# hassony2/homan

Measured on AMD Instinct MI355X. Metric: optimisation iters/sec (30-frame 256^2 clip), higher is better.
Workload: dtype f32

## Files before the change

homan_amd/csrc/raster_fwd.hip:

```cpp
#include "raster_ws.h"

#ifdef RASTER_TRACE
#define RASTER_TRACE_WGS 65536
__device__ unsigned g_raster_trace[RASTER_TRACE_WGS][9];
__device__ int g_raster_trace_F = 0, g_raster_trace_depth = -1;
#define RPH_MARK(k) do { if (tid == 0) { const unsigned long long t_ = wall_clock64(); rtr[k] += (unsigned)(t_ - rtr_t); rtr_t = t_; } } while (0)
#elif defined(RASTER_PHASES)
__device__ unsigned long long g_raster_ph[24];
#define RPH_MARK(k) do { if (tid == 0) { const unsigned long long t_ = clock64(); rph[k] += t_ - rph_t; rph_t = t_; } } while (0)
#else
#define RPH_MARK(k)
#endif
#ifndef CAND_CAP
#define CAND_CAP 512
#endif
#ifndef RB_PASS
#define RB_PASS 128
#endif
#ifndef HM_PRUNE
#define HM_PRUNE 1
#endif
#ifndef RASTER_WPE
#define RASTER_WPE 6
#endif
__device__ __forceinline__ void raster_fwd_body(
    const int blk, const float* __restrict__ faces9, const FaceBox* __restrict__ boxes, int B, int F, int S, float znear,
    float zfar, int* __restrict__ idx_map, unsigned short* __restrict__ alpha16, float* __restrict__ pooled,
    const float* __restrict__ keep, const float* __restrict__ ref, float* __restrict__ dimg,
    float* __restrict__ partials, const int* __restrict__ work_order, unsigned char* __restrict__ owned,
    float* __restrict__ pooled_depth, unsigned short* __restrict__ planes,
    int* __restrict__ bin_cnt, const int* __restrict__ bin_list, unsigned int* __restrict__ done, int reset_bins,
    unsigned char* __restrict__ region_state, int persistent, float* __restrict__ alpha_full, int mask_shared,
    float* __restrict__ dimg_full, const unsigned int* __restrict__ hint, unsigned long long* __restrict__ ts_slots,
    int* __restrict__ wo_dyn, unsigned int* __restrict__ wg_cost)
{
    const unsigned long long ts_t0 = (unsigned long long)wall_clock64();
    __shared__ unsigned long long zb[32 * 32];
    __shared__ int cand[2 * CAND_CAP];
    __shared__ float4 recs[RB_PASS][5];
    __shared__ int ustart[RB_PASS];
    __shared__ unsigned czn[RB_PASS];
    __shared__ unsigned hz[64];
    __shared__ unsigned short uq[RASTER_WAVES][128];
    __shared__ int wsum[RASTER_WAVES];
    __shared__ int cand_n[2];
    const int w = __builtin_amdgcn_readfirstlane((int)(threadIdx.x >> 6)), lane = threadIdx.x & 63, tid = threadIdx.x;
    const int is = 2 * S, tiles_x = S / HM_TILE, ntiles = tiles_x * tiles_x, regions_x = tiles_x / 2;
    const bool dyn = wo_dyn && hint[2] != 0u;
    const int wo = __builtin_amdgcn_readfirstlane(dyn ? wo_dyn[blk]
                                                     : work_order ? work_order[blk] : (int)(((blk % B) << 16) | (blk / B)));
    if (wo_dyn && !dyn && threadIdx.x == 0) wo_dyn[blk] = wo;
    const int region = wo & 0xffff, b = wo >> 16;
    const int rx = region % regions_x, ry = region / regions_x;
    const int tx = 2 * rx + (w & 1), ty = 2 * ry + (w >> 1);
    const int tile = ty * tiles_x + tx;

    const int gx0 = rx * 2 * HM_STILE, gx1 = gx0 + 2 * HM_STILE - 1;
    const int gy1 = is - 1 - ry * 2 * HM_STILE, gy0 = gy1 - (2 * HM_STILE - 1);
    const float gcx0 = (float)(2 * gx0 + 1 - is) / (float)is, gcx1 = (float)(2 * gx1 + 1 - is) / (float)is;
    const float gcy0 = (float)(2 * gy0 + 1 - is) / (float)is, gcy1 = (float)(2 * gy1 + 1 - is) / (float)is;
    const bool pow2 = (is & (is - 1)) == 0;
    const float inv_is = 1.0f / (float)is;
    const unsigned long long zb_empty = ((unsigned long long)__float_as_uint(zfar) << 32) | 0xffffffffull;

    int had_any = 0;
    const uint2* bx = reinterpret_cast<const uint2*>(boxes) + (long)b * F;
    const int nsx = (is + (1 << hm_sr_shift(is)) - 1) >> hm_sr_shift(is);
    const int sr = (gy0 >> hm_sr_shift(is)) * nsx + (gx0 >> hm_sr_shift(is));
    unsigned char* rstate = region_state + (long)b * regions_x * regions_x + region;
    const int nscan = bin_cnt ? bin_cnt[b * nsx * nsx + sr] : F;
    const int rstate0 = persistent ? (int)*rstate : 0;
    const int* scan = bin_cnt ? bin_list + ((long)b * nsx * nsx + sr) * F : nullptr;
    const bool idle = nscan == 0 && rstate0 == 1;
    const bool ts_on = hm_ts_enabled(hint) && tid == 0;
    if (ts_on) hm_ts_store(ts_slots, blk, 0, ts_t0);
#ifdef RASTER_TRACE
    unsigned rtr[6] = {0, 0, 0, 0, 0, 0}, rtr_cand = 0, rtr_units = 0;
    unsigned long long rtr_t = ts_t0;
#endif
#ifdef RASTER_PHASES
    unsigned long long rph[6] = {0, 0, 0, 0, 0, 0}, rph_t = clock64();
    unsigned long long rph_units[3] = {0, 0, 0};
    unsigned rph_pairs = 0;
    __shared__ unsigned s_rph_iters;
    if (tid == 0) s_rph_iters = 0u;
    __syncthreads();
#endif
    if (!idle) {
#pragma unroll
        for (int k = 0; k < 4; ++k) zb[tid + 256 * k] = zb_empty;
    }
    const int near_w = hint ? (int)(hint[0] & 1u) : 0;
    auto unit_body = [&](const int i, const int k) {
        const float4 r0 = recs[i][0], r1 = recs[i][1], r4 = recs[i][4];
        const int fn = __float_as_int(r4.z), pk = __float_as_int(r4.w);
        const int nbx = (pk >> 6) & 15;
        const int kby = (k * (pk >> 10)) >> 16;
        const int sx0 = 4 * ((pk & 7) + (k - kby * nbx)), sy0 = 4 * (((pk >> 3) & 7) + kby);
        float Xs[4], Ys[4];
#pragma unroll
        for (int j = 0; j < 4; ++j) {
            const int xi = gx0 + sx0 + j, yi = gy0 + sy0 + j;
            const float xn = (float)(2 * xi + 1 - is), yn = (float)(2 * yi + 1 - is);
            Xs[j] = pow2 ? xn * inv_is : xn / (float)is;
            Ys[j] = pow2 ? yn * inv_is : yn / (float)is;
        }
        unsigned acc[16];
        {
            const float vx[3] = {r0.x, r0.z, r1.x}, vy[3] = {r0.y, r0.w, r1.y};
#pragma unroll
            for (int e = 0; e < 3; ++e) {
                const int e1 = e == 2 ? 0 : e + 1;
                const float ex = vx[e1] - vx[e], ey = vy[e1] - vy[e];
                float rv[4], cv[4];
#pragma unroll
                for (int j = 0; j < 4; ++j) { rv[j] = (Ys[j] - vy[e]) * ex + 0.0f; cv[j] = (Xs[j] - vx[e]) * ey; }
#pragma unroll
                for (int idx = 0; idx < 16; ++idx) {
                    const unsigned d = __float_as_uint(rv[idx >> 2] - cv[idx & 3]);
                    acc[idx] = e ? (acc[idx] | d) : d;
                }
#pragma unroll
                for (int idx = 0; idx < 16; ++idx) asm volatile("" : "+v"(acc[idx]));
            }
        }
        unsigned outside = 0u;
#pragma unroll
        for (int idx = 15; idx >= 0; --idx) outside = __builtin_amdgcn_alignbit(outside, acc[idx], 31);
        unsigned inside = ~outside & 0xffffu;
        if (inside == 0u) return;
#if HM_PRUNE
        {
            const unsigned zn = czn[i];
#pragma unroll
            for (int j = 0; j < 4; ++j) {
                if (((inside >> (4 * j)) & 0xfu) == 0u) continue;
                const uint4 ka = *reinterpret_cast<const uint4*>(&zb[(sy0 + j) * 32 + sx0]);
                const uint4 kb = *reinterpret_cast<const uint4*>(&zb[(sy0 + j) * 32 + sx0 + 2]);
                unsigned keepm = (zn > ka.y ? 0u : 1u) | (zn > ka.w ? 0u : 2u) | (zn > kb.y ? 0u : 4u) | (zn > kb.w ? 0u : 8u);
                inside &= ~(0xfu << (4 * j)) | (keepm << (4 * j));
            }
            if (inside == 0u) return;
        }
#endif
#ifdef RASTER_PHASES
        rph_pairs += __popc(inside);
        {
            const unsigned mx = (unsigned)hm_wave_max((float)__popc(inside));
            if (lane == __ffsll((long long)__ballot(1)) - 1) atomicAdd(&s_rph_iters, mx);
        }
#endif
        const float4 r2 = recs[i][2], r3 = recs[i][3];
        const float rz0 = r1.z, rz1 = r1.w, rz2 = r2.x;
        const float iv[9] = {r2.y, r2.z, r2.w, r3.x, r3.y, r3.z, r3.w, r4.x, r4.y};
        const int xb = gx0 + sx0, yb = gy0 + sy0;
        while (inside) {
            const int sidx = __ffs((int)inside) - 1;
            inside &= inside - 1;
            const int j = sidx >> 2, c4 = sidx & 3;
            const float xf = (float)(xb + c4), yf = (float)(yb + j);
            float wgt[3], ws = 0.0f;
#pragma unroll
            for (int q = 0; q < 3; ++q) {
                float t = iv[3 * q] * xf;
                t = t + iv[3 * q + 1] * yf;
                t = t + iv[3 * q + 2];
                t = fminf(fmaxf(t, 0.0f), 1.0f);
                wgt[q] = t;
                ws += t;
            }
            float sum = wgt[0] * rz0;
            sum = sum + wgt[1] * rz1;
            sum = sum + wgt[2] * rz2;
            const float zp = ws / sum;
            if (zp > znear && zp < zfar)
                atomicMin(&zb[(sy0 + j) * 32 + sx0 + c4],
                          ((unsigned long long)__float_as_uint(zp) << 32) | (unsigned)fn);
        }
    };
    for (int cbase = 0; cbase < nscan; cbase += CAND_CAP) {
        if (tid == 0) { cand_n[0] = 0; cand_n[1] = 0; }
        __syncthreads();
        uint2 v[CAND_CAP / 256];
        int vf[CAND_CAP / 256];
#pragma unroll
        for (int k = 0; k < CAND_CAP / 256; ++k) {
            const int e = cbase + k * 256 + tid;
            vf[k] = e < nscan ? (scan ? scan[e] : e) : -1;
        }
#pragma unroll
        for (int k = 0; k < CAND_CAP / 256; ++k) v[k] = vf[k] >= 0 ? bx[vf[k]] : make_uint2(0u, 0u);
#pragma unroll
        for (int k = 0; k < CAND_CAP / 256; ++k) {
            const int fi = vf[k];
            const int x0 = v[k].x & 0x3fff, y0 = (int)(v[k].x >> 16), x1 = (int)(v[k].y & 0xffff), y1 = (int)(v[k].y >> 16);
            const unsigned m = (x1 < gx0 || x0 > gx1 || y1 < gy0 || y0 > gy1) ? 0u : ((v[k].x >> 14) & 3u);
#pragma unroll
            for (int var = 0; var < 2; ++var) {
                const bool hit = (m >> var) & 1u;
                const unsigned long long bal = __ballot(hit);
                if (bal == 0ull) continue;
                const int cls = var == near_w ? 0 : 1;
                int basep = 0;
                if (lane == 0) basep = atomicAdd(&cand_n[cls], __popcll(bal));
                basep = __builtin_amdgcn_readfirstlane(basep);
                const int at = basep + __popcll(bal & ((1ull << lane) - 1ull));
                if (hit) cand[cls ? 2 * CAND_CAP - 1 - at : at] = fi | (var << 30);
            }
        }
        __syncthreads();
        RPH_MARK(0);
        had_any |= cand_n[0] | cand_n[1];
        const int n_near = cand_n[0], n_far = cand_n[1];
        for (int e0 = 0; e0 < n_near || e0 < n_far; e0 += RB_PASS / 2) {
            int units = 0;
            const int cls = tid >> 6, ci = e0 + (tid & 63);
            if (tid < RB_PASS && ci < (cls ? n_far : n_near)) {
                const int e = cand[cls ? 2 * CAND_CAP - 1 - ci : ci];
                const int fi = e & 0x3fffffff, var = e >> 30;
                const float* src = faces9 + ((long)b * F + fi) * 9;
                const uint2 u = bx[fi];
                float f[9];
                if (var == 0) {
#pragma unroll
                    for (int k = 0; k < 9; ++k) f[k] = src[k];
                } else {
#pragma unroll
                    for (int k = 0; k < 3; ++k) { f[3 * k] = src[3 * (2 - k)]; f[3 * k + 1] = src[3 * (2 - k) + 1]; f[3 * k + 2] = src[3 * (2 - k) + 2]; }
                }
                float p[3][2];
#pragma unroll
                for (int k = 0; k < 3; ++k) { p[k][0] = topix(f[3 * k], is); p[k][1] = topix(f[3 * k + 1], is); }
                const float inv[9] = {
                    p[1][1] - p[2][1], p[2][0] - p[1][0], p[1][0] * p[2][1] - p[2][0] * p[1][1],
                    p[2][1] - p[0][1], p[0][0] - p[2][0], p[2][0] * p[0][1] - p[0][0] * p[2][1],
                    p[0][1] - p[1][1], p[1][0] - p[0][0], p[0][0] * p[1][1] - p[1][0] * p[0][1]};
                const float den = p[2][0] * (p[0][1] - p[1][1]) + p[0][0] * (p[1][1] - p[2][1]) +
                                  p[1][0] * (p[2][1] - p[0][1]);
                bool miss = (den == 0.0f);
#pragma unroll
                for (int k = 0; k < 3; ++k) {
                    const int k1 = (k + 1) % 3;
                    const float ax = f[3 * k], ay = f[3 * k + 1], ex = f[3 * k1] - ax, ey = f[3 * k1 + 1] - ay;
                    bool all_out = true;
                    float mag = 0.f;
                    float lhs[4], rhs[4];
#pragma unroll
                    for (int cnr = 0; cnr < 4; ++cnr) {
                        const float X = (cnr & 1) ? gcx1 : gcx0, Y = (cnr & 2) ? gcy1 : gcy0;
                        lhs[cnr] = (Y - ay) * ex;
                        rhs[cnr] = (X - ax) * ey;
                        mag = fmaxf(mag, fabsf(lhs[cnr]) + fabsf(rhs[cnr]));
                    }
#pragma unroll
                    for (int cnr = 0; cnr < 4; ++cnr) all_out = all_out && (lhs[cnr] < rhs[cnr] - 1e-5f * mag);
                    miss = miss || all_out;
                }
                if (!miss) {
                    const int x0 = u.x & 0x3fff, y0 = (int)(u.x >> 16), x1 = (int)(u.y & 0xffff), y1 = (int)(u.y >> 16);
                    const int bx0 = (max(x0, gx0) - gx0) >> 2, bx1 = (min(x1, gx1) - gx0) >> 2;
                    const int by0 = (max(y0, gy0) - gy0) >> 2, by1 = (min(y1, gy1) - gy0) >> 2;
                    const int nbx = bx1 - bx0 + 1;
                    units = nbx * (by1 - by0 + 1);
                    const float rz0 = 1.0f / f[2], rz1 = 1.0f / f[5], rz2 = 1.0f / f[8];
                    recs[tid][0] = make_float4(f[0], f[1], f[3], f[4]);
                    recs[tid][1] = make_float4(f[6], f[7], rz0, rz1);
                    recs[tid][2] = make_float4(rz2, inv[0] / den, inv[1] / den, inv[2] / den);
                    recs[tid][3] = make_float4(inv[3] / den, inv[4] / den, inv[5] / den, inv[6] / den);
                    recs[tid][4] = make_float4(inv[7] / den, inv[8] / den, __int_as_float(fi + var * F),
                                               __int_as_float(bx0 | (by0 << 3) | (nbx << 6) | (((0x10000 + nbx - 1) / nbx) << 10)));
                    czn[tid] = __float_as_uint((1.0f / fmaxf(rz0, fmaxf(rz1, rz2))) * (1.0f - 1e-5f));
                }
            }
            const int incl = hm_wave_scan_incl(units);
            if (lane == 63 && w < 2) wsum[w] = incl;
            if (tid < RB_PASS) ustart[tid] = incl - units;
            __syncthreads();
            const int total_near = wsum[0], total_far = wsum[1];
#ifdef RASTER_TRACE
            rtr_cand += (unsigned)min(n_near - e0, RB_PASS / 2) * (e0 < n_near) + ((unsigned)min(n_far - e0, RB_PASS / 2) * (e0 < n_far) << 16);
            rtr_units += (unsigned)total_near + ((unsigned)total_far << 16);
#endif
#ifdef RASTER_PHASES
            if (tid < RB_PASS && ci < (cls ? n_far : n_near)) atomicAdd(&g_raster_ph[12 + cls], 1ull);
            rph_units[0] += total_near;
            rph_units[1] += total_far;
#endif
            RPH_MARK(1);
            for (int u = tid; u < total_near; u += 256) {
                int i = 0;
#pragma unroll
                for (int stp = RB_PASS / 4; stp > 0; stp >>= 1)
                    if (ustart[i + stp] <= u) i += stp;
                unit_body(i, u - ustart[i]);
            }
            RPH_MARK(2);
            if (total_far > 0) {
                if (tid < 64) hz[tid] = 0u;
                __syncthreads();
                {
                    const int blk = tid >> 2, row = (blk >> 3) * 4 + (tid & 3), col0 = (blk & 7) * 4;
                    const uint4 ka = *reinterpret_cast<const uint4*>(&zb[row * 32 + col0]);
                    const uint4 kb = *reinterpret_cast<const uint4*>(&zb[row * 32 + col0 + 2]);
                    atomicMax(&hz[blk], max(max(ka.y, ka.w), max(kb.y, kb.w)));
                }
                __syncthreads();
                RPH_MARK(3);
                int qn = 0;
                for (int u0 = 64 * w; u0 < total_far; u0 += 256) {
                    const int u = u0 + lane;
                    bool pass = false;
                    int ent = 0;
                    if (u < total_far) {
                        int i = 0;
#pragma unroll
                        for (int stp = RB_PASS / 4; stp > 0; stp >>= 1)
                            if (ustart[RB_PASS / 2 + i + stp] <= u) i += stp;
                        i += RB_PASS / 2;
                        const int k = u - ustart[i];
                        const int pk = __float_as_int(recs[i][4].w);
                        const int nbx = (pk >> 6) & 15, kby = (k * (pk >> 10)) >> 16;
                        const int blk = (((pk >> 3) & 7) + kby) * 8 + (pk & 7) + (k - kby * nbx);
                        pass = !(czn[i] > hz[blk]);
                        ent = i | (k << 8);
                    }
                    const unsigned long long bal = __ballot(pass);
#ifdef RASTER_PHASES
                    if (lane == 0) atomicAdd(&g_raster_ph[21], (unsigned long long)__popcll(bal));
#endif
                    if (pass) uq[w][qn + __popcll(bal & ((1ull << lane) - 1ull))] = (unsigned short)ent;
                    qn += __popcll(bal);
                    wave_sync();
                    if (qn >= 64) {
                        qn -= 64;
                        const int e = uq[w][qn + lane];
                        wave_sync();
                        unit_body(e & 0xff, e >> 8);
                    }
                }
                if (lane < qn) {
                    const int e = uq[w][lane];
                    unit_body(e & 0xff, e >> 8);
                }
            }
            __syncthreads();
            RPH_MARK(4);
        }
    }
    __syncthreads();
    if (tid == 0 && bin_cnt && reset_bins) {
        const int per_side = (1 << hm_sr_shift(is)) / (2 * HM_STILE);
        const int rw = min(per_side, regions_x - per_side * (gx0 >> hm_sr_shift(is))), rh = min(per_side, regions_x - per_side * (gy0 >> hm_sr_shift(is)));
        const int slot = b * nsx * nsx + sr;
        if (atomicAdd(done + slot, 1u) == (unsigned)(rw * rh) - 1u) {
            bin_cnt[slot] = 0;
            atomicExch(done + slot, 0u);
        }
    }

    if (persistent && !had_any && rstate0 == 1) {
#ifdef RASTER_PHASES
        if (tid == 0) atomicAdd(&g_raster_ph[7], 1ull);
#endif
        if (wg_cost && tid == 0) wg_cost[blk] = 0u;
        return;
    }
    __syncthreads();
    if (tid == 0) *rstate = (persistent && !had_any) ? 1 : 0;

    const int r = ty * HM_TILE + (lane >> 3), c = tx * HM_TILE + (lane & 7);
    const int xi0 = 2 * c, yi0 = is - 1 - 2 * r;
    float zmin[4];
    int imin[4];
#pragma unroll
    for (int s4 = 0; s4 < 4; ++s4) {
        const int dy = s4 >> 1, dx = s4 & 1;
        const unsigned long long key = zb[(yi0 - dy - gy0) * 32 + (xi0 + dx - gx0)];
        zmin[s4] = __uint_as_float((unsigned)(key >> 32));
        imin[s4] = (int)(unsigned)(key & 0xffffffffull);
    }

    int* im = idx_map + (long)b * is * is;
#pragma unroll
    for (int dy = 0; dy < 2; ++dy) {
        hm_out_store2(im + (long)(yi0 - dy) * is + xi0, imin[2 * dy], imin[2 * dy + 1]);
    }
#pragma unroll
    for (int s = 0; s < 4; ++s) {
        const int left = __builtin_amdgcn_update_dpp(-2, imin[s], 0x138, 0xf, 0xf, false);
        const int up = __builtin_amdgcn_ds_bpermute(((lane - 8) & 63) << 2, imin[s]);
        if (imin[s] >= 0 && (s == 0 || imin[s] != imin[s - 1]) && imin[s] != left && (lane < 8 || imin[s] != up))
            owned[(long)b * 2 * F + imin[s]] = 1;
    }
    const Ballots4 bal = {__ballot(imin[0] >= 0), __ballot(imin[1] >= 0), __ballot(imin[2] >= 0), __ballot(imin[3] >= 0)};
    if (lane < 16) {
        const int rr = lane >> 1, dy = lane & 1;
        const unsigned long long be = dy ? bal.s2 : bal.s0, bo = dy ? bal.s3 : bal.s1;
        const unsigned a = (unsigned)(be >> (8 * rr)) & 0xffu;
        const unsigned o = (unsigned)(bo >> (8 * rr)) & 0xffu;
        const unsigned word = spread8(a) | (spread8(o) << 1);
        alpha16[(((long)b * (is / 16) + ty) * (is / 16) + tx) * 16 + lane] = (unsigned short)word;
    }
    const int cnt = (imin[0] >= 0) + (imin[1] >= 0) + (imin[2] >= 0) + (imin[3] >= 0);
    const float pool = 0.25f * (float)cnt;
    const long po = ((long)b * S + r) * S + c;
    hm_out_store(pooled + po, pool);
    if (alpha_full) {
#pragma unroll
        for (int dy = 0; dy < 2; ++dy)
            *reinterpret_cast<float2*>(alpha_full + ((long)b * is + 2 * r + dy) * is + xi0) =
                make_float2(imin[2 * dy] >= 0 ? 1.f : 0.f, imin[2 * dy + 1] >= 0 ? 1.f : 0.f);
    }
    if (pooled_depth) pooled_depth[po] = (((zmin[0] + zmin[1]) + zmin[2]) + zmin[3]) / 4.0f;
    if (partials && dimg_full) {
        const float* kb = keep + ((mask_shared & 1) ? 0 : (long)b * is * is);
        const float* rb = ref + ((mask_shared & 1) ? 0 : (long)b * is * is);
        const bool ps_store = !(mask_shared & 2);
        float sqs = 0.f, ins = 0.f, uns = 0.f;
        unsigned long long nq[4], pq[4];
#pragma unroll
        for (int dy = 0; dy < 2; ++dy) {
            const long at = (long)(2 * r + dy) * is + xi0;
            const float2 k2 = *reinterpret_cast<const float2*>(kb + at), r2 = *reinterpret_cast<const float2*>(rb + at);
            const float i0 = k2.x * (imin[2 * dy] >= 0 ? 1.f : 0.f), i1 = k2.y * (imin[2 * dy + 1] >= 0 ? 1.f : 0.f);
            const float d0 = i0 - r2.x, d1 = i1 - r2.y;
            const float g0 = k2.x * d0, g1 = k2.y * d1;
            if (ps_store) *reinterpret_cast<float2*>(dimg_full + (long)b * is * is + at) = make_float2(g0, g1);
            sqs += d0 * d0 + d1 * d1;
            ins += i0 * r2.x + i1 * r2.y;
            uns += fminf(fmaxf(i0 + r2.x, 0.0f), 1.0f) + fminf(fmaxf(i1 + r2.y, 0.0f), 1.0f);
            nq[2 * dy] = __ballot(g0 < 0.0f); pq[2 * dy] = __ballot(g0 > 0.0f);
            nq[2 * dy + 1] = __ballot(g1 < 0.0f); pq[2 * dy + 1] = __ballot(g1 > 0.0f);
        }
        const Ballots4 nbv = {nq[0], nq[1], nq[2], nq[3]}, pbv = {pq[0], pq[1], pq[2], pq[3]};
        emit_planes(bal, nbv, pbv, b, B, is, tx, ty, lane, planes);
        const float sq = hm_wave_sum(sqs), inter = hm_wave_sum(ins), uni = hm_wave_sum(uns);
        if (lane == 0) {
            float* o = partials + ((long)b * ntiles + tile) * 4;
            o[0] = sq; o[1] = inter; o[2] = uni; o[3] = 0.f;
        }
    } else if (partials) {
        const long pm = (mask_shared & 1) ? (long)r * S + c : po;
        const float kp = keep[pm], rf = ref[pm];
        const float image = kp * pool;
        const float diff = image - rf;
        hm_out_store(dimg + po, kp * diff);
        {
            const unsigned long long nb1 = __ballot(kp * diff < 0.0f), pb1 = __ballot(kp * diff > 0.0f);
            const Ballots4 nbv = {nb1, nb1, nb1, nb1}, pbv = {pb1, pb1, pb1, pb1};
            emit_planes(bal, nbv, pbv, b, B, is, tx, ty, lane, planes);
        }
        const float sq = hm_wave_sum(diff * diff);
        const float inter = hm_wave_sum(image * rf);
        const float uni = hm_wave_sum(fminf(fmaxf(image + rf, 0.0f), 1.0f));
        if (lane == 0) {
            float* o = partials + ((long)b * ntiles + tile) * 4;
            o[0] = sq; o[1] = inter; o[2] = uni; o[3] = 0.f;
        }
    }
    if (ts_on) hm_ts_store(ts_slots, blk, 1, (unsigned long long)wall_clock64());
    if (wg_cost && tid == 0) wg_cost[blk] = (unsigned)min((unsigned long long)wall_clock64() - ts_t0, 0xfffffffeull) + 1u;
#ifdef RASTER_TRACE
    RPH_MARK(5);
    if (tid == 0 && blk < RASTER_TRACE_WGS && (g_raster_trace_F == 0 || g_raster_trace_F == F) &&
        (g_raster_trace_depth < 0 || g_raster_trace_depth == (pooled_depth ? 1 : 0))) {
        unsigned* o = g_raster_trace[blk];
        for (int k = 0; k < 6; ++k) o[k] = rtr[k];
        o[6] = (unsigned)ts_t0; o[7] = rtr_cand; o[8] = rtr_units;
    }
#endif
#ifdef RASTER_PHASES
    RPH_MARK(5);
    if (tid == 0) {
        for (int k = 0; k < 6; ++k) atomicAdd(&g_raster_ph[k], rph[k]);
        atomicAdd(&g_raster_ph[6], 1ull);
        atomicAdd(&g_raster_ph[8], rph_units[0]);
        atomicAdd(&g_raster_ph[9], rph_units[1]);
    }
    {
        const unsigned wp = (unsigned)hm_wave_sum((float)rph_pairs);
        if (lane == 0) atomicAdd(&g_raster_ph[11], (unsigned long long)wp);
        __syncthreads();
        if (tid == 0) atomicAdd(&g_raster_ph[10], (unsigned long long)s_rph_iters);
    }
#endif
}

__global__ __launch_bounds__(64 * RASTER_WAVES) __attribute__((amdgpu_waves_per_eu(RASTER_WPE, 8))) void k_raster_fwd(RasterFwdK a)
{
    HM_CHAIN_KERNEL();
    raster_fwd_body((int)blockIdx.x, a.faces9, a.boxes, a.B, a.F, a.S, a.znear, a.zfar, a.idx_map, a.alpha16, a.pooled, a.keep, a.ref,
                    a.dimg, a.partials, a.work_order, a.owned, a.pooled_depth, a.planes, a.bin_cnt, a.bin_list, a.done, a.reset_bins,
                    a.region_state, a.persistent, a.alpha_full, a.mask_shared, a.dimg_full, a.hint, a.ts_slots, a.wo_dyn, a.wg_cost);
}
__global__ __launch_bounds__(64 * RASTER_WAVES) __attribute__((amdgpu_waves_per_eu(RASTER_WPE, 8))) void k_raster_fwd_multi(RasterFwdMulti m)
{
    HM_CHAIN_KERNEL();
    int g = 0;
#pragma unroll
    for (int k = 1; k < HM_MAX_RENDERS; ++k) g += (k < m.n && (int)blockIdx.x >= m.first[k]) ? 1 : 0;
    g = __builtin_amdgcn_readfirstlane(g);
    const RasterFwdK& a = m.r[g];
    raster_fwd_body((int)blockIdx.x - m.first[g], a.faces9, a.boxes, a.B, a.F, a.S, a.znear, a.zfar, a.idx_map, a.alpha16, a.pooled, a.keep,
                    a.ref, a.dimg, a.partials, a.work_order, a.owned, a.pooled_depth, a.planes, a.bin_cnt, a.bin_list, a.done,
                    a.reset_bins, a.region_state, a.persistent, a.alpha_full, a.mask_shared, a.dimg_full, a.hint, a.ts_slots,
                    a.wo_dyn, a.wg_cost);
}


__global__ __launch_bounds__(256) void k_sil_reduce(const float* __restrict__ partials, int B, int ntiles,
                                                     const float* __restrict__ keep_sum, float* __restrict__ frame_rec,
                                                     float* __restrict__ out, float* __restrict__ frame_out, int clip_len,
                                                     int out_stride)
{
    HM_LATENCY_KERNEL();
    sil_reduce_frame(blockIdx.x, partials, ntiles, keep_sum, frame_rec, out, frame_out, clip_len, out_stride);
}

__global__ __launch_bounds__(256) void k_shade_rgb(const int* __restrict__ idx_map, const float* __restrict__ verts,
                                                   const int* __restrict__ faces, int faces_bstride,
                                                   const float* __restrict__ textures, int B, int V, int F, int S,
                                                   float dx, float dy, float dz, float amb, float dirw, float bg0,
                                                   float bg1, float bg2, float* __restrict__ rgb)
{
    const int b = blockIdx.y, pix = blockIdx.x * 256 + threadIdx.x;
    if (pix >= S * S) return;
    const int r = pix / S, c = pix - r * S, is = 2 * S;
    const int* idx = idx_map + (long)b * is * is;
    float acc[3] = {0.f, 0.f, 0.f};
#pragma unroll
    for (int q = 0; q < 4; ++q) {
        const int yi = is - 1 - (2 * r + (q >> 1)), xi = 2 * c + (q & 1);
        const int fn = idx[(long)yi * is + xi];
        float col[3] = {bg0, bg1, bg2};
        if (fn >= 0) {
            const int f = fn >= F ? fn - F : fn;
            const int* fc = faces + (long)b * faces_bstride + 3 * f;
            const float* v0 = verts + ((long)b * V + fc[0]) * 3;
            const float* v1 = verts + ((long)b * V + fc[1]) * 3;
            const float* v2 = verts + ((long)b * V + fc[2]) * 3;
            const float a[3] = {v0[0] - v1[0], v0[1] - v1[1], v0[2] - v1[2]};
            const float e[3] = {v2[0] - v1[0], v2[1] - v1[1], v2[2] - v1[2]};
            float n[3] = {a[1] * e[2] - a[2] * e[1], a[2] * e[0] - a[0] * e[2], a[0] * e[1] - a[1] * e[0]};
            const float len = fmaxf(sqrtf(n[0] * n[0] + n[1] * n[1] + n[2] * n[2]), 1e-5f);
            float cs = (n[0] / len) * dx + (n[1] / len) * dy + (n[2] / len) * dz;
            if (fn >= F) cs = -cs;
            const float light = amb + dirw * fmaxf(cs, 0.f);
            const float* t = textures + ((long)b * F + f) * 3;
            col[0] = t[0] * light; col[1] = t[1] * light; col[2] = t[2] * light;
        }
        acc[0] += col[0]; acc[1] += col[1]; acc[2] += col[2];
    }
#pragma unroll
    for (int ch = 0; ch < 3; ++ch) rgb[(((long)b * 3 + ch) * S + r) * S + c] = 0.25f * acc[ch];
}

static RasterFwdK raster_fwd_k(const SilWs& w, const RasterFwdArgs& a)
{
    RasterFwdK k = {w.faces9, w.boxes, a.B, a.F, a.S, a.znear, a.zfar, w.idx_map, w.alpha16, a.pooled, a.keep, a.ref, w.dimg,
                    a.fused ? w.partials : (float*)nullptr, a.work_order, w.owned, a.pooled_depth, w.planes, a.bins,
                    w.bin_list, w.bin_done, a.reset_bins, w.region_state, a.persistent, a.alpha_full, a.mask_shared,
                    a.per_sample_grad ? w.gimg : (float*)nullptr, w.counter + 24, w.ts, a.reorder ? w.wo_dyn : (int*)nullptr,
                    a.reorder ? w.wg_cost : (unsigned int*)nullptr};
    return k;
}
void hm_launch_raster_fwd(const SilWs& w, const RasterFwdArgs& a, hipStream_t stream)
{
    const int ntiles = (a.S / 8) * (a.S / 8);
    hipLaunchKernelGGL(k_raster_fwd, dim3(a.B * (ntiles / RASTER_WAVES)), dim3(64 * RASTER_WAVES), a.lds_pad, stream,
                       raster_fwd_k(w, a));
}
void hm_launch_raster_fwd_multi(const SilWs* w, const RasterFwdArgs* a, int n, hipStream_t stream)
{
    RasterFwdMulti m;
    m.n = n;
    int at = 0;
    for (int g = 0; g < HM_MAX_RENDERS; ++g) {
        const int q = g < n ? g : n - 1;
        m.r[g] = raster_fwd_k(w[q], a[q]);
        m.first[g] = at;
        if (g < n) at += a[g].B * ((a[g].S / 8) * (a[g].S / 8) / RASTER_WAVES);
    }
    m.first[HM_MAX_RENDERS] = at;
    hipLaunchKernelGGL(k_raster_fwd_multi, dim3(at), dim3(64 * RASTER_WAVES), a[0].lds_pad, stream, m);
}
void hm_launch_sil_reduce(const SilWs& w, int B, int S, const float* keep_sum, float* loss_out, float* frame_out, int clip_len,
                          int out_stride, hipStream_t stream)
{
    hipLaunchKernelGGL(k_sil_reduce, dim3(B), dim3(256), 0, stream, w.partials, B, (S / 8) * (S / 8), keep_sum, w.frame_rec,
                       loss_out, frame_out, clip_len, out_stride);
}
void hm_launch_shade_rgb(const SilWs& w, const float* verts, const int* faces, int faces_bstride, const float* textures, int B,
                         int V, int F, int S, const float* light_dir, float amb, float dirw, const float* background, float* rgb,
                         hipStream_t stream)
{
    hipLaunchKernelGGL(k_shade_rgb, dim3(hm_cdiv((long)S * S, 256), B), dim3(256), 0, stream, w.idx_map, verts, faces,
                       faces_bstride, textures, B, V, F, S, light_dir[0], light_dir[1], light_dir[2], amb, dirw, background[0],
                       background[1], background[2], rgb);
}
int hm_raster_fwd_occupancy(int* blocks_per_cu)
{
    return hipOccupancyMaxActiveBlocksPerMultiprocessor(blocks_per_cu, k_raster_fwd, 64 * RASTER_WAVES, 0) == hipSuccess ? HM_OK
                                                                                                                        : HM_ERR_LAUNCH;
}
#ifdef RASTER_TRACE
extern "C" int hm_debug_raster_trace_filter(int F, int depth)
{
    (void)hipMemcpyToSymbol(HIP_SYMBOL(g_raster_trace_F), &F, sizeof(int));
    (void)hipMemcpyToSymbol(HIP_SYMBOL(g_raster_trace_depth), &depth, sizeof(int));
    return HM_OK;
}
extern "C" int hm_debug_raster_trace(unsigned* out, int nwg)
{
    (void)hipDeviceSynchronize();
    const size_t bytes = sizeof(unsigned) * 9 * (size_t)min(nwg, RASTER_TRACE_WGS);
    (void)hipMemcpyFromSymbol(out, HIP_SYMBOL(g_raster_trace), bytes);
    void* dev = nullptr;
    (void)hipGetSymbolAddress(&dev, HIP_SYMBOL(g_raster_trace));
    (void)hipMemset(dev, 0, sizeof(unsigned) * 9 * RASTER_TRACE_WGS);
    return HM_OK;
}
#endif
#ifdef RASTER_PHASES
extern "C" int hm_debug_raster_phases(unsigned long long* out)
{
    unsigned long long z[24] = {0};
    (void)hipDeviceSynchronize();
    (void)hipMemcpyFromSymbol(out, HIP_SYMBOL(g_raster_ph), sizeof(z));
    (void)hipMemcpyToSymbol(HIP_SYMBOL(g_raster_ph), z, sizeof(z));
    return HM_OK;
}
#endif
```

Baseline: 6628.

## Replace per-face block rectangles with per-row triangle span masks

Instead of enumerating every 4x4 pixel block inside a face's clipped bounding rectangle, each face record now stores a 64-bit mask of blocks that the triangle's edges can actually cover, computed per block row with conservative slack. Unit enumeration and the hierarchical-z pass decode block coordinates from the mask with popcounts. This is meant to cut empty unit evaluations for thin or diagonal triangles. In exchange, setup per face gets costlier, decoding per unit gets slightly heavier, and the slack-based conservative test risks dropping edge pixels if it is too tight.

```diff
diff --git a/homan_amd/csrc/raster_fwd.hip b/homan_amd/csrc/raster_fwd.hip
--- a/homan_amd/csrc/raster_fwd.hip
+++ b/homan_amd/csrc/raster_fwd.hip
@@ -1,4 +1,5 @@
 #include "raster_ws.h"
+#include "raster_spans.h"
 
 #ifdef RASTER_TRACE
 #define RASTER_TRACE_WGS 65536
@@ -38,7 +39,8 @@
     __shared__ unsigned long long zb[32 * 32];
     __shared__ int cand[2 * CAND_CAP];
     __shared__ float4 recs[RB_PASS][5];
-    __shared__ int ustart[RB_PASS];
+    __shared__ unsigned short ustart[RB_PASS];
+    __shared__ unsigned span_hi[RB_PASS];
     __shared__ unsigned czn[RB_PASS];
     __shared__ unsigned hz[64];
     __shared__ unsigned short uq[RASTER_WAVES][128];
@@ -82,6 +84,7 @@
     unsigned long long rph[6] = {0, 0, 0, 0, 0, 0}, rph_t = clock64();
     unsigned long long rph_units[3] = {0, 0, 0};
     unsigned rph_pairs = 0;
+    unsigned rph_empty = 0;
     __shared__ unsigned s_rph_iters;
     if (tid == 0) s_rph_iters = 0u;
     __syncthreads();
@@ -93,10 +96,10 @@
     const int near_w = hint ? (int)(hint[0] & 1u) : 0;
     auto unit_body = [&](const int i, const int k) {
         const float4 r0 = recs[i][0], r1 = recs[i][1], r4 = recs[i][4];
-        const int fn = __float_as_int(r4.z), pk = __float_as_int(r4.w);
-        const int nbx = (pk >> 6) & 15;
-        const int kby = (k * (pk >> 10)) >> 16;
-        const int sx0 = 4 * ((pk & 7) + (k - kby * nbx)), sy0 = 4 * (((pk >> 3) & 7) + kby);
+        const int fn = __float_as_int(r4.z);
+        int brow, bcol;
+        hm_span_decode(__float_as_uint(r4.w), span_hi[i], k, &brow, &bcol);
+        const int sx0 = 4 * bcol, sy0 = 4 * brow;
         float Xs[4], Ys[4];
 #pragma unroll
         for (int j = 0; j < 4; ++j) {
@@ -128,6 +131,9 @@
 #pragma unroll
         for (int idx = 15; idx >= 0; --idx) outside = __builtin_amdgcn_alignbit(outside, acc[idx], 31);
         unsigned inside = ~outside & 0xffffu;
+#ifdef RASTER_PHASES
+        rph_empty += inside == 0u ? 1u : 0u;
+#endif
         if (inside == 0u) return;
 #if HM_PRUNE
         {
@@ -260,21 +266,25 @@
                     const int x0 = u.x & 0x3fff, y0 = (int)(u.x >> 16), x1 = (int)(u.y & 0xffff), y1 = (int)(u.y >> 16);
                     const int bx0 = (max(x0, gx0) - gx0) >> 2, bx1 = (min(x1, gx1) - gx0) >> 2;
                     const int by0 = (max(y0, gy0) - gy0) >> 2, by1 = (min(y1, gy1) - gy0) >> 2;
-                    const int nbx = bx1 - bx0 + 1;
-                    units = nbx * (by1 - by0 + 1);
                     const float rz0 = 1.0f / f[2], rz1 = 1.0f / f[5], rz2 = 1.0f / f[8];
                     recs[tid][0] = make_float4(f[0], f[1], f[3], f[4]);
                     recs[tid][1] = make_float4(f[6], f[7], rz0, rz1);
                     recs[tid][2] = make_float4(rz2, inv[0] / den, inv[1] / den, inv[2] / den);
                     recs[tid][3] = make_float4(inv[3] / den, inv[4] / den, inv[5] / den, inv[6] / den);
-                    recs[tid][4] = make_float4(inv[7] / den, inv[8] / den, __int_as_float(fi + var * F),
-                                               __int_as_float(bx0 | (by0 << 3) | (nbx << 6) | (((0x10000 + nbx - 1) / nbx) << 10)));
+                    recs[tid][4] = make_float4(inv[7] / den, inv[8] / den, __int_as_float(fi + var * F), 0.0f);
                     czn[tid] = __float_as_uint((1.0f / fmaxf(rz0, fmaxf(rz1, rz2))) * (1.0f - 1e-5f));
+                    unsigned mlo, mhi;
+                    units = hm_span_mask(f, is, gx0, gy0, bx0, bx1, by0, by1, &mlo, &mhi);
+#ifdef RASTER_PHASES
+                    atomicAdd(&g_raster_ph[23], (unsigned long long)((bx1 - bx0 + 1) * (by1 - by0 + 1)));
+#endif
+                    recs[tid][4].w = __uint_as_float(mlo);
+                    span_hi[tid] = mhi;
                 }
             }
             const int incl = hm_wave_scan_incl(units);
             if (lane == 63 && w < 2) wsum[w] = incl;
-            if (tid < RB_PASS) ustart[tid] = incl - units;
+            if (tid < RB_PASS) ustart[tid] = (unsigned short)(incl - units);
             __syncthreads();
             const int total_near = wsum[0], total_far = wsum[1];
 #ifdef RASTER_TRACE
@@ -318,9 +328,9 @@
                             if (ustart[RB_PASS / 2 + i + stp] <= u) i += stp;
                         i += RB_PASS / 2;
                         const int k = u - ustart[i];
-                        const int pk = __float_as_int(recs[i][4].w);
-                        const int nbx = (pk >> 6) & 15, kby = (k * (pk >> 10)) >> 16;
-                        const int blk = (((pk >> 3) & 7) + kby) * 8 + (pk & 7) + (k - kby * nbx);
+                        int brow, bcol;
+                        hm_span_decode(__float_as_uint(recs[i][4].w), span_hi[i], k, &brow, &bcol);
+                        const int blk = brow * 8 + bcol;
                         pass = !(czn[i] > hz[blk]);
                         ent = i | (k << 8);
                     }
@@ -480,6 +490,8 @@
     {
         const unsigned wp = (unsigned)hm_wave_sum((float)rph_pairs);
         if (lane == 0) atomicAdd(&g_raster_ph[11], (unsigned long long)wp);
+        const unsigned we = (unsigned)hm_wave_sum((float)rph_empty);
+        if (lane == 0) atomicAdd(&g_raster_ph[22], (unsigned long long)we);
         __syncthreads();
         if (tid == 0) atomicAdd(&g_raster_ph[10], (unsigned long long)s_rph_iters);
     }
diff --git a/homan_amd/csrc/raster_spans.h b/homan_amd/csrc/raster_spans.h
--- /dev/null
+++ b/homan_amd/csrc/raster_spans.h
@@ -0,0 +1,75 @@
+#pragma once
+#include <math.h>
+#if defined(__HIPCC__)
+#define HM_SPAN_FN __host__ __device__ __forceinline__
+#else
+#define HM_SPAN_FN static inline
+#endif
+#if defined(__clang__)
+#define HM_SPAN_UNROLL _Pragma("unroll")
+#else
+#define HM_SPAN_UNROLL
+#endif
+
+#define HM_SPAN_ABS_SLACK 0.01f
+#define HM_SPAN_REL_SLACK 1e-5f
+#define HM_SPAN_MAX_T 1e6f
+
+HM_SPAN_FN int hm_span_mask(const float* f, int is, int gx0, int gy0, int bx0, int bx1, int by0, int by1, unsigned* lo,
+                            unsigned* hi)
+{
+    const float fis = (float)is;
+    float c[3], s[3];
+    unsigned upm = 0u;
+    HM_SPAN_UNROLL
+    for (int k = 0; k < 3; ++k) {
+        const int k1 = k == 2 ? 0 : k + 1;
+        const float ax = f[3 * k], ay = f[3 * k + 1];
+        const float ex = f[3 * k1] - ax, ey = f[3 * k1 + 1] - ay;
+        const float xa = 0.5f * (ax * fis + (fis - 1.0f)), ya = 0.5f * (ay * fis + (fis - 1.0f));
+        const float sl = ey != 0.0f ? ex / ey : 0.0f;
+        const float T = fabsf(xa) + fis + (fabsf(ya) + fis) * fabsf(sl);
+        const bool use = ey != 0.0f && T < HM_SPAN_MAX_T;
+        const float sg = ey < 0.0f ? -1.0f : 1.0f;
+        const float slack = HM_SPAN_ABS_SLACK + HM_SPAN_REL_SLACK * T;
+        s[k] = use ? sg * sl : 0.0f;
+        c[k] = use ? sg * (xa - ya * sl) + slack : 3e38f;
+        upm |= (use && ey < 0.0f) ? 0u : 1u << k;
+    }
+    unsigned long long m = 0ull;
+    int n = 0;
+    for (int r = by0; r <= by1; ++r) {
+        const float ya = (float)(gy0 + 4 * r), yb = ya + 3.0f;
+        float xlo = (float)(gx0 + 4 * bx0), xhi = (float)(gx0 + 4 * bx1 + 3);
+        HM_SPAN_UNROLL
+        for (int k = 0; k < 3; ++k) {
+            const float v = fmaxf(c[k] + ya * s[k], c[k] + yb * s[k]);
+            const bool up = (upm >> k) & 1u;
+            xhi = up ? fminf(xhi, v) : xhi;
+            xlo = up ? xlo : fmaxf(xlo, -v);
+        }
+        if (!(xlo <= xhi)) continue;
+        const int i0 = (int)ceilf(xlo), i1 = (int)floorf(xhi);
+        if (i0 > i1) continue;
+        const int b0 = (i0 - gx0) >> 2, b1 = (i1 - gx0) >> 2;
+        m |= (unsigned long long)((2u << b1) - (1u << b0)) << (8 * r);
+        n += b1 - b0 + 1;
+    }
+    *lo = (unsigned)m;
+    *hi = (unsigned)(m >> 32);
+    return n;
+}
+
+HM_SPAN_FN void hm_span_decode(unsigned lo, unsigned hi, int k, int* row, int* col)
+{
+    const int nlo = __builtin_popcount(lo);
+    const int top = k >= nlo;
+    const unsigned w = top ? hi : lo;
+    const int kk = top ? k - nlo : k;
+    const int c1 = __builtin_popcount(w & 0xffu), c2 = __builtin_popcount(w & 0xffffu), c3 = __builtin_popcount(w & 0xffffffu);
+    const int r = (kk >= c1) + (kk >= c2) + (kk >= c3);
+    const int before = r == 0 ? 0 : r == 1 ? c1 : r == 2 ? c2 : c3;
+    const unsigned byte = (w >> (8 * r)) & 0xffu;
+    *row = r + 4 * top;
+    *col = __builtin_ctz(byte | 0x100u) + (kk - before);
+}
```

New measurement: 6618, median of 3. Within noise of the previous version (-0.2%).
